# BenLangmead/bowtie2

Measured on NVIDIA H100. Metric: Mreads/s, higher is better.
Workload: dtype u64 popcount (FM rank) + s16x2 DPX (DP)

## Files before the change

### bowtie2_b200/csrc/xengine.cu

```cuda
#include <new>
#include <mutex>
#include <map>
#include <cstdio>
#include <cstddef>
#include <chrono>
#include <cstring>
#include <string>
#include <vector>
#include "dp_ungapped_device.cuh"
#include "dp_device.cuh"
#define XE_HD __device__
#include "xengine.cuh"
#include "xengine_shared.h"

template <typename OFF> int launch_dp_e2e(const DevIndex<OFF> &, const bt2g_scoring &, const DpLaunch &, int, cudaStream_t);
template <typename OFF> int launch_dp_local(const DevIndex<OFF> &, const bt2g_scoring &, const DpLaunch &, int, cudaStream_t);
template <typename OFF> void launch_exact_sweep2(const DevIndex<OFF> &, const uint64_t *, uint64_t, int, int, uint8_t *, uint64_t *, const uint64_t *, const uint32_t *, unsigned long long *, int, cudaStream_t, unsigned long long *, int);
void launch_pack_reads(const uint8_t *, const uint64_t *, uint64_t, int, uint64_t *, uint32_t *, cudaStream_t);
template <typename OFF> void launch_one_mm_sel(const DevIndex<OFF> &, const uint8_t *, const uint8_t *, const uint64_t *, uint64_t, const uint32_t *, const int32_t *, const uint8_t *, const bt2g_scoring &, int, bt2g_mm_hit *, int32_t *, cudaStream_t, bool);
template <typename OFF> void launch_seed_search_active(const DevIndex<OFF> &, const uint64_t *, uint64_t, int, int, const int32_t *, const int32_t *, const uint8_t *, uint64_t *, int32_t *, const uint64_t *, const uint32_t *, unsigned long long *, int, cudaStream_t);

extern "C" int bt2g_policy_align(const bt2g_policy_backend *, const bt2g_policy_params *, const bt2g_reads *, const char *const *,
                                 bt2g_read_result *, uint8_t *, uint32_t, bt2g_pair_result *, uint64_t *);

namespace {
using namespace xe;

#define XE_MM_MAXHITS 16
#define XE_TEV 96

struct XQueues {
	uint32_t nDpA, nDpM, nMm, nSeed, nDone, nFallback, nActive, pad1;
	unsigned long long cellsA, cellsM;
};

struct DpOut { bt2g_dp_problem *probs; bt2g_dp_summary *summ; bt2g_dp_cand *cands; bt2g_dp_aln *alns; uint8_t *ops; int maxCands, maxAlns, maxOps; };

struct XDev {
	const uint8_t *seq, *qual; const uint64_t *roff;
	const uint32_t *seeds;
	const uint64_t *packed; const uint32_t *nmask;
	const uint8_t *mine; const uint64_t *ee;
	const bt2g_mm_hit *mmHits; const int32_t *mmCounts;
	uint32_t *mmSel; int32_t *mmMinsc; uint8_t *mmMask;
	const uint64_t *ranges; const int32_t *nseeds; int maxSeeds;
	int32_t *seedInterval, *seedOffset; uint8_t *seedActive;
	DpOut A, M;
	XQueues *q;
	XUnit *units; uint8_t *status; uint64_t nUnits;
	bt2g_read_result *res; uint8_t *resOps; bt2g_pair_result *pairs; uint32_t resMaxOps;
};

template <typename OFF, bool K>
struct DevSvc {
	static constexpr bool kReport = K;
	const DevIndex<OFF> &ix; const bt2g_scoring &sc; const XDev &d;
	__device__ DevSvc(const DevIndex<OFF> &i, const bt2g_scoring &s, const XDev &dd) : ix(i), sc(s), d(dd) {}
	__device__ const uint8_t *codes(int read) const { return d.seq + d.roff[read]; }
	__device__ const uint8_t *quals(int read) const { return d.qual + d.roff[read]; }
	__device__ int rdlen(int read) const { return (int)(d.roff[read + 1] - d.roff[read]); }
	__device__ uint32_t randSeed(int read) const { return d.seeds[read]; }
	__device__ void sweep(int read, int mined[2], uint64_t tb[4]) const {
		mined[0] = d.mine[2 * (size_t)read]; mined[1] = d.mine[2 * (size_t)read + 1];
		for(int j = 0; j < 4; j++) tb[j] = d.ee[4 * (size_t)read + j];
	}
	__device__ int mmMax() const { return XE_MM_MAXHITS; }
// ... 44 lines not shown
	if(names) {
		const char *nm = names + i * (uint64_t)nameStride;
		for(uint32_t k = 0; k < nameStride && nm[k]; k++) { if(nm[k] == '/') break; rseed ^= (uint32_t)(unsigned char)nm[k] << ((k & 3) << 3); }
	} else {
		char buf[24]; int n = 0;
		uint64_t v = paired ? i >> 1 : i;
		char tmp[20]; int t = 0;
		do { tmp[t++] = (char)('0' + v % 10); v /= 10; } while(v);
		buf[n++] = 'r';
		while(t) buf[n++] = tmp[--t];
		for(int k = 0; k < n; k++) rseed ^= (uint32_t)(unsigned char)buf[k] << ((k & 3) << 3);
	}
	out[i] = rseed;
}

__global__ void k_xe_reset(XUnit *units, uint8_t *status, uint64_t nUnits, int paired) {
	const uint64_t i = blockIdx.x * (uint64_t)blockDim.x + threadIdx.x;
	if(i >= nUnits) return;
	x_unit_reset(units[i], (uint32_t)i, paired != 0);
	status[i] = 0;
}

__device__ __forceinline__ uint32_t agg_inc(uint32_t *ctr) {
	const unsigned act = __activemask();
	const unsigned peers = __match_any_sync(act, (unsigned long long)ctr);
	const int lane = threadIdx.x & 31, leader = __ffs(peers) - 1;
	uint32_t base = 0;
	if(lane == leader) base = atomicAdd(ctr, (uint32_t)__popc(peers));
	base = __shfl_sync(peers, base, leader);
	return base + (uint32_t)__popc(peers & ((1u << lane) - 1u));
}

template <typename OFF, int MINB, bool K>
__global__ void __launch_bounds__(128, MINB) k_xe_step(DevIndex<OFF> ix, bt2g_scoring sc, XParams P, XDev d, const uint32_t *activeIn, uint32_t *activeOut,
                                                       uint32_t nAct, int spread) {
	const uint64_t tt = blockIdx.x * (uint64_t)blockDim.x + threadIdx.x;
	const uint64_t t = tt >> spread;
	const bool valid = t < nAct && (tt & ((1u << spread) - 1u)) == 0;
	const uint64_t i = valid ? (activeIn ? activeIn[t] : t) : 0;
	int r = XR_DONE;
	if(valid) {
		XUnit &u = d.units[i];
		DevSvc<OFF, K> svc(ix, sc, d);
		r = x_step(P, u, svc);
		switch(r) {
		case XR_DP: case XR_DP_MATE: {
			const bool mate = r == XR_DP_MATE;
			const uint32_t slot = agg_inc(mate ? &d.q->nDpM : &d.q->nDpA);
			(mate ? d.M : d.A).probs[slot] = u.rqProb;
			u.dpSlot = (int32_t)slot;
			const unsigned long long cells = (unsigned long long)svc.rdlen((int)u.rqProb.read_idx) * (unsigned long long)(u.rqProb.refr - u.rqProb.refl + 1);
			atomicAdd(mate ? &d.q->cellsM : &d.q->cellsA, cells);
			break; }
		case XR_ONE_MM: {
			const uint32_t slot = agg_inc(&d.q->nMm);
			d.mmSel[slot] = (uint32_t)u.rqRead; d.mmMinsc[slot] = u.rqMinsc; d.mmMask[slot] = (uint8_t)((u.rqNofw ? 0 : 1) | (u.rqNorc ? 0 : 2));
			u.dpSlot = (int32_t)slot;
			break; }
		case XR_SEED:
			d.seedActive[u.rqRead] = 1; d.seedInterval[u.rqRead] = u.rqInterval; d.seedOffset[u.rqRead] = u.rqOffset;
			agg_inc(&d.q->nSeed);
			break;
		case XR_DONE: {
			d.status[i] = 1;
			agg_inc(&d.q->nDone);
			if(K) break;
			const uint64_t r0 = u.paired ? 2 * i : i; const int nr = u.paired ? 2 : 1;
			for(int k = 0; k < nr; k++) x_fill_result(u, k, svc.codes((int)(r0 + k)), d.res[r0 + k], d.resOps + (r0 + k) * (uint64_t)d.resMaxOps, d.resMaxOps);
			if(u.paired) { bt2g_pair_result pr; pr.pair_type = u.pairType; pr.kind = u.pairKind; pr.source = 0; pr.score_sum = (int32_t)u.scoreSum; pr.fraglen = u.fraglen; d.pairs[i] = pr; }
			break; }
		default:
			d.status[i] = 2;
			agg_inc(&d.q->nFallback);
			break;
		}
	}
	__syncwarp();
	const bool cont = valid && (r == XR_DP || r == XR_DP_MATE || r == XR_ONE_MM || r == XR_SEED);
	const unsigned m = __ballot_sync(0xffffffffu, cont);
	if(m) {
		const int lane = threadIdx.x & 31, leader = __ffs(m) - 1;
		uint32_t base = 0;
		if(lane == leader) base = atomicAdd(&d.q->nActive, (uint32_t)__popc(m));
		base = __shfl_sync(0xffffffffu, base, leader);
		if(cont) activeOut[base + (uint32_t)__popc(m & ((1u << lane) - 1u))] = (uint32_t)i;
	}
}

__global__ void __launch_bounds__(128) k_xe_report(XParams P, const XUnit *units, const uint8_t *status, uint64_t nUnits, const uint8_t *seq,
                                                   const uint64_t *roff, uint32_t maxPer, bt2g_read_result *res, uint8_t *ops, uint32_t maxOps,
                                                   bt2g_pair_result *pairs, uint32_t *nEntries, uint32_t *truncated) {
	const uint64_t w = (blockIdx.x * (uint64_t)blockDim.x + threadIdx.x) >> 5;
	const int lane = threadIdx.x & 31;
	if(w >= nUnits || status[w] != 1) return;
	const XUnit &u = units[w];
	const int n = x_report_count(u, P), nw = n < (int)maxPer ? n : (int)maxPer;
	if(lane == 0) {
		nEntries[w] = (uint32_t)nw;
		if(n > (int)maxPer && maxPer > 1) atomicOr(truncated, 1u);
	}
	const int per = u.paired ? 2 : 1;
	const uint64_t r0 = w * (uint64_t)per;
	const uint8_t *c0 = seq + roff[r0], *c1 = u.paired ? seq + roff[r0 + 1] : nullptr;
	for(int e = lane; e < (nw > 1 ? nw : 1); e += 32) {
		const uint64_t ent = w * (uint64_t)maxPer + (uint64_t)e;
		x_report_entry(u, P, e, c0, c1, res + ent * per, ops + ent * per * (uint64_t)maxOps, maxOps, u.paired ? pairs + ent : nullptr);
	}
}

struct DpWork {
	DpOut o{}; uint8_t *codes = nullptr; int32_t *lastH = nullptr; uint64_t *rawKeys = nullptr;
	int maxCol = 0, packed = 0, maxRaw = 0; uint64_t codeStride = 0, chunk = 0, numSlots = 0;
};

}

struct bt2g_xengine {
	bt2g_ctx *ctx = nullptr;
	bt2g_policy_params pp{};
	bt2g_scoring sc{};
	XParams P{}; XTables T;
	uint64_t maxUnits = 0, maxReads = 0, maxBases = 0; int maxLen = 0; uint32_t maxOps = 0;
	std::vector<void *> allocs;
	int32_t *dTabs = nullptr;
	XDev d{};
	DpWork A, M;
	uint64_t *packed = nullptr; uint32_t *nmask = nullptr; unsigned long long *nextTask = nullptr;
	uint32_t *active[2] = {nullptr, nullptr};
	uint8_t *dSeq = nullptr, *dQual = nullptr; uint64_t *dOff = nullptr; char *dNames = nullptr; uint32_t nameStrideCap = 0;
	XQueues *hq = nullptr;
	uint8_t *hStatus = nullptr;
	int sms = 148;
	cudaStream_t stream = nullptr;
	cudaStream_t streamHi = nullptr;
	bool ownStreams = false;
	int debug = 0;
	int bigSpread = 0;
	int stepOcc = 4;
	uint64_t stats[8] = {0, 0, 0, 0, 0, 0, 0, 0};
	float stageMs[12] = {0, 0, 0, 0, 0, 0, 0, 0, 0, 0, 0, 0};
	cudaEvent_t tev[2][XE_TEV]; int tevN[2] = {0, 0};
	cudaEvent_t evJoin = nullptr; int dpSideBySide = 1;
	uint64_t launches = 0;
	uint32_t maxPer = 0;
	bt2g_read_result *kRes = nullptr; uint8_t *kOps = nullptr; bt2g_pair_result *kPairs = nullptr; uint32_t *kN = nullptr, *kTrunc = nullptr;
	cudaEvent_t ev[8] = {nullptr, nullptr, nullptr, nullptr, nullptr, nullptr, nullptr, nullptr};
};

namespace {

template <typename T> int xalloc(bt2g_xengine *e, T *&ptr, uint64_t count) {
	void *v = nullptr;
	const cudaError_t err = cudaMalloc(&v, (count ? count : 1) * sizeof(T));
	if(err != cudaSuccess) { e->ctx->err = std::string("xengine cudaMalloc: ") + cudaGetErrorString(err); return -2; }
	e->allocs.push_back(v);
	ptr = (T *)v;
	return 0;
}

int setupDp(bt2g_xengine *e, DpWork &w, int maxCol, uint64_t cap, int maxCands, int maxAlns) {
	const bt2g_scoring &sc = e->sc;
// ... 28 lines not shown
	const DevIndex<OFF> ix = bt2g_dev_index<OFF>(e->ctx);
	e->launches += (!e->sc.local && w.packed == 3) ? 2 * ((n + w.chunk - 1) / w.chunk) : 1;
	return e->sc.local ? launch_dp_local<OFF>(ix, e->sc, L, e->maxLen, st) : launch_dp_e2e<OFF>(ix, e->sc, L, e->maxLen, st);
}

template <typename OFF>
int runBatch(bt2g_xengine *e, uint64_t nReads, const char *dNames, uint32_t nameStride, cudaStream_t st0) {
	cudaStream_t st = st0;
	bt2g_ctx *ctx = e->ctx;
	const bool paired = e->P.paired != 0;
	const uint64_t nUnits = paired ? nReads / 2 : nReads;
	const DevIndex<OFF> ix = bt2g_dev_index<OFF>(ctx);
	XDev &d = e->d;
	d.nUnits = nUnits;
	d.packed = e->packed; d.nmask = e->nmask;
	const unsigned T = 128;
	auto grid = [&](uint64_t m, unsigned t) { return (unsigned)((m + t - 1) / t); };
	for(int k = 0; k < 8; k++) e->stats[k] = 0;
	for(int k = 0; k < 12; k++) e->stageMs[k] = 0.f;
	e->tevN[0] = e->tevN[1] = 0;
	e->launches = 4;
	cudaEvent_t *ev = e->ev;
	auto lap = [&](int a, int b, int stage) { float ms = 0.f; if(cudaEventElapsedTime(&ms, ev[a], ev[b]) == cudaSuccess) e->stageMs[stage] += ms; };
	cudaEventRecord(ev[7], st);
	k_xe_seeds<<<grid(nReads, T), T, 0, st>>>(d.seq, d.qual, d.roff, nReads, dNames, nameStride, paired ? 1 : 0, e->P.seed, const_cast<uint32_t *>(d.seeds));
	k_xe_reset<<<grid(nUnits, T), T, 0, st>>>(d.units, d.status, nUnits, paired ? 1 : 0);
	launch_pack_reads(d.seq, d.roff, nReads, e->maxLen, e->packed, e->nmask, st);
	launch_exact_sweep2<OFF>(ix, d.roff, nReads, 0, 0, const_cast<uint8_t *>(d.mine), const_cast<uint64_t *>(d.ee), e->packed, e->nmask, e->nextTask, e->sms, st, nullptr,
	                         ix.extText ? 2 : 0 );
	BT2G_CUDA_TRY(ctx, cudaMemsetAsync(d.seedActive, 0, nReads, st));
	BT2G_CUDA_TRY(ctx, cudaGetLastError());
	uint64_t done = 0;
	uint32_t nActive = 0;
	cudaEventRecord(ev[0], st);
	for(uint64_t wave = 0;; wave++) {
		BT2G_CUDA_TRY(ctx, cudaMemsetAsync(d.q, 0, sizeof(XQueues), st));
		{
			const uint32_t nAct = wave == 0 ? (uint32_t)nUnits : nActive;
			const uint32_t *in = wave == 0 ? nullptr : e->active[wave & 1];
			uint32_t *out = e->active[(wave + 1) & 1];
			const int spread = (uint64_t)nAct * 32 <= (uint64_t)e->sms * 2048 * 4 ? 5 : e->bigSpread;
			const uint64_t nThr = (uint64_t)nAct << spread;
			if(e->maxPer) k_xe_step<OFF, 4, true><<<grid(nThr, 128), 128, 0, st>>>(ix, e->sc, e->P, d, in, out, nAct, spread);
			else if(e->stepOcc >= 8) k_xe_step<OFF, 8, false><<<grid(nThr, 128), 128, 0, st>>>(ix, e->sc, e->P, d, in, out, nAct, spread);
			else if(e->stepOcc >= 6) k_xe_step<OFF, 6, false><<<grid(nThr, 128), 128, 0, st>>>(ix, e->sc, e->P, d, in, out, nAct, spread);
			else k_xe_step<OFF, 4, false><<<grid(nThr, 128), 128, 0, st>>>(ix, e->sc, e->P, d, in, out, nAct, spread);
		}
		cudaEventRecord(ev[1], st);
		e->launches++;
		BT2G_CUDA_TRY(ctx, cudaMemcpyAsync(e->hq, d.q, sizeof(XQueues), cudaMemcpyDeviceToHost, st));
		BT2G_CUDA_TRY(ctx, cudaStreamSynchronize(st));
		if(wave == 0) lap(7, 0, 0); else { lap(2, 3, 2); lap(3, 4, 3); lap(4, 5, 4); lap(5, 0, 5); }
		for(int qi = 0; qi < 2; qi++) {
			for(int k = 0; k + 1 < e->tevN[qi]; k++) { float ms = 0.f; if(cudaEventElapsedTime(&ms, e->tev[qi][k], e->tev[qi][k + 1]) == cudaSuccess) e->stageMs[8 + (k & 1)] += ms; }
			e->tevN[qi] = 0;
		}
		lap(0, 1, 1);
		const XQueues q = *e->hq;
		if(e->debug) {
			float ms = 0.f; cudaEventElapsedTime(&ms, ev[0], ev[1]);
			fprintf(stderr, "[xengine] wave %llu: step %.3f ms; done %u fallback %u | dpA %u dpM %u mm %u seed %u\n", (unsigned long long)wave, ms, q.nDone, q.nFallback,
			        q.nDpA, q.nDpM, q.nMm, q.nSeed);
		}
		e->stats[0]++; e->stats[1] += q.nFallback; e->stats[2] += q.nDpA; e->stats[3] += q.nDpM; e->stats[4] += q.cellsA; e->stats[5] += q.cellsM;
		e->stats[6] += q.nMm; e->stats[7] += q.nSeed;
		e->launches += (q.nMm ? 1 : 0) + (q.nSeed ? 1 : 0);
		done += q.nDone + q.nFallback;
		nActive = q.nActive;
		if(done >= nUnits) break;
		if(e->ownStreams) st = (uint64_t)nActive * 32 <= (uint64_t)e->sms * 2048 * 4 ? e->streamHi : e->stream;
		if(q.nDpA + q.nDpM + q.nMm + q.nSeed == 0) { ctx->err = "xengine: units neither finished nor waiting"; return -5; }
		cudaEventRecord(ev[2], st);
		if(q.nMm) launch_one_mm_sel<OFF>(ix, d.seq, d.qual, d.roff, q.nMm, d.mmSel, d.mmMinsc, d.mmMask, e->sc, XE_MM_MAXHITS, const_cast<bt2g_mm_hit *>(d.mmHits), const_cast<int32_t *>(d.mmCounts), st,
		                                      ix.extText != 0);
		cudaEventRecord(ev[3], st);
		if(q.nSeed) {
			launch_seed_search_active<OFF>(ix, d.roff, nReads, e->P.seedLen, d.maxSeeds, d.seedInterval, d.seedOffset, d.seedActive, const_cast<uint64_t *>(d.ranges),
			                               const_cast<int32_t *>(d.nseeds), e->packed, e->nmask, e->nextTask, e->sms, st);
			BT2G_CUDA_TRY(ctx, cudaMemsetAsync(d.seedActive, 0, nReads, st));
		}
		cudaEventRecord(ev[4], st);
		const bool sideBySide = e->ownStreams && e->dpSideBySide && q.nDpA && q.nDpM && (uint64_t)(q.nDpA + q.nDpM) * 16 <= (uint64_t)e->sms * 2048;
		cudaStream_t stM = sideBySide ? (st == e->stream ? e->streamHi : e->stream) : st;
		if(launchDp<OFF>(e, e->A, q.nDpA, st)) { ctx->err = "xengine: DP launch rejected"; return -1; }
		cudaEventRecord(ev[5], st);
		if(launchDp<OFF>(e, e->M, q.nDpM, stM)) { ctx->err = "xengine: DP launch rejected"; return -1; }
		if(sideBySide) { cudaEventRecord(e->evJoin, stM); cudaStreamWaitEvent(st, e->evJoin, 0); }
		cudaEventRecord(ev[0], st);
		BT2G_CUDA_TRY(ctx, cudaGetLastError());
	}
	lap(7, 1, 7);
	return 0;
}

}

static int createEngine(bt2g_ctx *ctx, const bt2g_policy_params *pp, uint64_t maxUnits, uint32_t maxLen, uint32_t maxPer, bt2g_xengine **out) {
	BT2G_CUDA_TRY(ctx, cudaSetDevice(ctx->device));
	if(maxPer) {
		const uint64_t per = pp->paired ? 2 : 1, ents = maxUnits * (uint64_t)maxPer;
		const uint64_t need = ents * per * (sizeof(bt2g_read_result) + maxLen + 80) + (pp->paired ? ents * sizeof(bt2g_pair_result) : 0) + maxUnits * 4;
		size_t freeB = 0, totalB = 0;
		BT2G_CUDA_TRY(ctx, cudaMemGetInfo(&freeB, &totalB));
		if(need > freeB) {
			char msg[200];
			snprintf(msg, sizeof msg, "xengine: the -k / -a report arrays (%.2f GiB for %llu units x %u entries) do not fit the device's free memory (%.2f GiB)",
			         need / 1073741824.0, (unsigned long long)maxUnits, maxPer, freeB / 1073741824.0);
			ctx->err = msg;
			return -2;
		}
	}
	bt2g_xengine *e = new(std::nothrow) bt2g_xengine();
	if(!e) return -4;
	e->ctx = ctx; e->pp = *pp; e->maxLen = (int)maxLen; e->maxUnits = maxUnits;
	e->maxReads = pp->paired ? 2 * maxUnits : maxUnits; e->maxBases = e->maxReads * (uint64_t)maxLen;
	e->maxOps = maxLen + 80;
	cudaDeviceGetAttribute(&e->sms, cudaDevAttrMultiProcessorCount, ctx->device);
	if(const char *o = getenv("BT2G_XE_OCC")) e->stepOcc = atoi(o);
	if(getenv("BT2G_XE_DEBUG")) e->debug = 1;
	if(const char *o = getenv("BT2G_XE_DP_SERIAL")) e->dpSideBySide = atoi(o) ? 0 : 1;
	if(const char *o = getenv("BT2G_XE_SPREAD")) { e->bigSpread = atoi(o); if(e->bigSpread < 0 || e->bigSpread > 5) e->bigSpread = 0; }
	scoringFromParams(pp, &e->sc);
	ctx->scoring = e->sc;
	buildParams(pp, ctx->info.off_size, (int)maxLen, e->P, e->T);
	int rc = 0;
	const uint64_t nR = e->maxReads, nU = maxUnits;
	rc |= xalloc(e, e->dTabs, 4ull * (maxLen + 1));
	XDev &d = e->d;
	rc |= xalloc(e, e->dSeq, e->maxBases); rc |= xalloc(e, e->dQual, e->maxBases); rc |= xalloc(e, e->dOff, nR + 1);
	uint32_t *seeds; uint8_t *mine; uint64_t *ee;
	rc |= xalloc(e, seeds, nR); rc |= xalloc(e, mine, nR * 2); rc |= xalloc(e, ee, nR * 4);
	d.seeds = seeds; d.mine = mine; d.ee = ee;
	bt2g_mm_hit *mmHits; int32_t *mmCounts;
	rc |= xalloc(e, mmHits, nU * 4 * XE_MM_MAXHITS); rc |= xalloc(e, mmCounts, nU * 4);
	d.mmHits = mmHits; d.mmCounts = mmCounts;
	rc |= xalloc(e, d.mmSel, nU); rc |= xalloc(e, d.mmMinsc, nU); rc |= xalloc(e, d.mmMask, nU);
	{
		int minIval = 1 << 30;
		for(int l = 1; l <= (int)maxLen; l++) { minIval = std::min(minIval, std::min(e->T.ivalOne[l], e->T.ivalBoth[l])); }
		int ms = 1 + ((int)maxLen - std::min<int>(pp->seed_len, (int)maxLen)) / std::max(1, minIval) + 1;
		if(ms > XE_MAX_SEEDS) ms = XE_MAX_SEEDS + 1;
		d.maxSeeds = ms;
	}
	uint64_t *ranges; int32_t *nseeds;
	rc |= xalloc(e, ranges, nR * 2ull * d.maxSeeds * 4); rc |= xalloc(e, nseeds, nR);
	d.ranges = ranges; d.nseeds = nseeds;
	rc |= xalloc(e, d.seedInterval, nR); rc |= xalloc(e, d.seedOffset, nR); rc |= xalloc(e, d.seedActive, nR);
	rc |= xalloc(e, e->packed, (e->maxBases >> 5) + nR + 2); rc |= xalloc(e, e->nmask, (e->maxBases >> 5) + nR + 2); rc |= xalloc(e, e->nextTask, 1);
	rc |= xalloc(e, d.q, 1); rc |= xalloc(e, d.units, nU); rc |= xalloc(e, d.status, nU);
	rc |= xalloc(e, e->active[0], nU); rc |= xalloc(e, e->active[1], nU);
	if(maxPer) {
		const uint64_t ents = nU * (uint64_t)maxPer, rows = ents * (pp->paired ? 2 : 1);
		e->maxPer = maxPer;
		rc |= xalloc(e, e->kRes, rows); rc |= xalloc(e, e->kOps, rows * (uint64_t)e->maxOps); rc |= xalloc(e, e->kN, nU); rc |= xalloc(e, e->kTrunc, 1);
		if(pp->paired) rc |= xalloc(e, e->kPairs, ents);
		d.res = nullptr; d.resOps = nullptr; d.pairs = nullptr;
	} else {
		rc |= xalloc(e, d.res, nR); rc |= xalloc(e, d.resOps, nR * (uint64_t)e->maxOps); rc |= xalloc(e, d.pairs, nU);
	}
	d.resMaxOps = e->maxOps;
	if(!rc) {
		const int maxColA = (int)maxLen + 4 * 15 + 4;
		int gapMax = 15;
		for(int l = 1; l <= (int)maxLen; l++) { gapMax = std::max(gapMax, std::max(e->P.maxReadGaps(e->T.minsc[l], l), e->P.maxRefGaps(e->T.minsc[l], l))); }
		if(gapMax > 512) gapMax = 512;
		const uint64_t maxfrag = std::max<uint64_t>(pp->pe.maxfrag, maxLen);
		int maxColM = (int)std::min<uint64_t>(maxfrag + 2ull * maxLen + 2ull * gapMax + 16, 8000);
		const int maxCands = e->sc.local ? 16384 : 256, maxAlns = e->sc.local ? 32 : 8;
		rc |= setupDp(e, e->A, maxColA, nU, maxCands, maxAlns);
		if(pp->paired) rc |= setupDp(e, e->M, maxColM, nU, maxCands, maxAlns);
		else e->M = e->A;
		d.A = e->A.o; d.M = e->M.o;
	}
	cudaError_t err = cudaSuccess;
	if(!rc) {
		std::vector<int32_t> tabs(4ull * (maxLen + 1));
		for(uint32_t l = 0; l <= maxLen; l++) { tabs[l] = e->T.minsc[l]; tabs[(maxLen + 1) + l] = e->T.nceilRaw[l]; tabs[2 * (maxLen + 1) + l] = e->T.ivalOne[l]; tabs[3 * (maxLen + 1) + l] = e->T.ivalBoth[l]; }
		err = cudaMemcpy(e->dTabs, tabs.data(), tabs.size() * 4, cudaMemcpyHostToDevice);
		e->P.minscTab = e->dTabs; e->P.nceilRawTab = e->dTabs + (maxLen + 1); e->P.ivalOneTab = e->dTabs + 2 * (maxLen + 1); e->P.ivalBothTab = e->dTabs + 3 * (maxLen + 1);
		if(err == cudaSuccess) err = cudaHostAlloc((void **)&e->hq, sizeof(XQueues), cudaHostAllocDefault);
		if(err == cudaSuccess) err = cudaHostAlloc((void **)&e->hStatus, nU, cudaHostAllocDefault);
		for(int k = 0; k < 8 && err == cudaSuccess; k++) err = cudaEventCreate(&e->ev[k]);
		for(int k = 0; k < 2 * XE_TEV && err == cudaSuccess; k++) err = cudaEventCreate(&e->tev[k / XE_TEV][k % XE_TEV]);
// ... 263 lines not shown
```

### bowtie2_b200/csrc/xengine.cuh

```cuda
#pragma once
#include <stdint.h>
#include "../../include/bt2g.h"
#include "mapq_device.cuh"
#include "pe_device.cuh"

#ifndef XE_HD
#define XE_HD __host__ __device__
#endif
#define XE_HH __host__ __device__

namespace xe {

#define XE_MIN_I64 (-9223372036854775807LL - 1)
#define XE_BIG ((int64_t)1 << 62)
enum { EXHAUSTED = 1, FULFILLED, PERFECT, SOFT_LIMIT, HARD_LIMIT };
enum { XR_DONE = 0, XR_ONE_MM = 1, XR_SEED = 2, XR_DP = 3, XR_DP_MATE = 4, XR_FALLBACK = 5 };

#define XE_MAX_LEN    512
#define XE_ARENA      12288
#define XE_SEEN_IV    224
#define XE_EXR        8
#define XE_MM1        24
#define XE_MAX_SEEDS  64
#define XE_SATS       (2 * XE_MAX_SEEDS)
// ... 1337 lines not shown
			XE_CALL_EXT(5, stepExtUnpaired);
			if(u.xRet == FULFILLED) { if(u.usDone) u.rdone = 1; }
			else if(u.xRet == PERFECT || u.xRet == HARD_LIMIT) u.rdone = 1;
			if(!u.rdone && c.shNelt / c.shNonz < 300) u.rdone = 1;
		}
		finishRead();
		u.doneFlag = 1;
		return XR_DONE;
	}
	}
	XE_FB(u);
	return XR_FALLBACK;
}

template <typename Svc>
XE_HD void XEngine<Svc>::finishRead() {
	if(u.nus == 0) return;
	XSel buf[XE_LIST];
	for(int i = 0; i < u.nus; i++) { buf[i].score = x_aln(u, u.usAlns[i])->score; buf[i].idx = i; }
	x_select(buf, u.nus, u.rnd);
	u.resAligned[0] = 1; u.resAln[0] = u.usAlns[buf[0].idx];
	u.resHasXs[0] = u.nus > 1; u.resXs[0] = u.nus > 1 ? buf[1].score : 0;
	u.resMapq[0] = (int)mapq(x_aln(u, u.resAln[0])->score, u.resHasXs[0] != 0, u.resXs[0], P.minScore(u.m[0].rdlen), u.m[0].perfect);
	if(Svc::kReport && !P.mmode) x_permute_selected(buf, u.nus, u.usAlns, nullptr);
}

template <typename Svc>
XE_HD inline int x_step(const XParams &P, XUnit &u, Svc &svc) {
	XEngine<Svc> e(P, u, svc);
	const int r = u.paired ? e.stepPair() : e.stepRead();
	if(u.fallback) return XR_FALLBACK;
	return r;
}
XE_HD inline void x_unit_reset(XUnit &u, uint32_t id, bool paired) {
	u.pc = 0; u.pcExt = 0; u.fallback = 0; u.paired = paired; u.doneFlag = 0; u.id = id; u.arenaTop = 0; u.cur = 0;
	u.nents = 0; u.nsats = 0; u.nrands = 0; u.nseenPool = 0; u.nhitl = 0; u.natt = 0; u.attCursor = 0; u.dpSlot = -1;
	u.pairType = 0; u.pairKind = 5; u.scoreSum = 0; u.fraglen = 0;
	for(int k = 0; k < 2; k++) { u.resAligned[k] = 0; u.resHasXs[k] = 0; u.resMapq[k] = 0; u.resXs[k] = 0; u.resAln[k] = 0xffff; }
}

XE_HD inline void x_fill_row(const XAln *a, bool hasXs, int64_t xs, int mapq, const uint8_t *codes, bt2g_read_result &out, uint8_t *ops, uint32_t maxOps) {
	out.found = 0; out.score = 0; out.score2 = INT32_MIN; out.fw = 0; out.tidx = 0; out.refoff = 0; out.nops = 0; out.ndp = 0;
	out.trim_left = out.trim_right = 0; out.mapq = 0; out.pad = 0;
	if(!a) return;
	const int nops = x_aln_to_ops(a, codes, ops, maxOps);
	out.found = (a->nedits == 0 && a->ext() == a->rdlen) ? 2 : 1;
	out.score = a->score; if(hasXs) out.score2 = (int32_t)xs;
	out.fw = a->fw; out.tidx = (uint64_t)a->tidx; out.refoff = a->refoff; out.nops = nops;
	out.trim_left = a->trimLeft(); out.trim_right = a->rdlen - a->ext() - a->trimLeft();
	out.mapq = mapq; out.pad = a->refns;
}
XE_HD inline void x_fill_result(const XUnit &u, int k, const uint8_t *codes, bt2g_read_result &out, uint8_t *ops, uint32_t maxOps) {
	x_fill_row(u.resAligned[k] ? x_aln(u, u.resAln[k]) : nullptr, u.resHasXs[k] != 0, u.resXs[k], u.resMapq[k], codes, out, ops, maxOps);
}

XE_HD inline int x_report_secondaries(const XUnit &u, const XParams &P, int n) {
	if(P.mmode || n < 1) return 0;
	return (int)((int64_t)n < P.khits ? (int64_t)n : P.khits) - 1;
}
XE_HD inline int x_report_count(const XUnit &u, const XParams &P) {
	if(!u.paired) return u.resAligned[0] ? 1 + x_report_secondaries(u, P, u.nus) : 0;
	if(u.pairType == 1) return 1 + x_report_secondaries(u, P, u.nrs12);
	const int s0 = u.resAligned[0] ? x_report_secondaries(u, P, u.nrs1u) : 0, s1 = u.resAligned[1] ? x_report_secondaries(u, P, u.nrs2u) : 0;
	if(s0 + s1 == 0) return 1;
	return (u.resAligned[0] ? 1 + s0 : 1) + (u.resAligned[1] ? 1 + s1 : 1);
}
// ... 33 lines not shown
```

### bowtie2_b200/csrc/xengine_host.cpp

```cpp
#include <cmath>
#include <cstring>
#include <string>
#include <vector>
#include "../../include/bt2g.h"
#define __host__
#define __device__
#define __forceinline__ inline
#include "xengine.cuh"
#include "xengine_shared.h"

namespace xe {

static double funcF(int type, double C, double L, double x) {
	const double g = type == 1 ? 0.0 : type == 2 ? x : type == 3 ? std::sqrt(x) : std::log(x);
	return C + L * g;
}

void buildParams(const bt2g_policy_params *pp, int offSize, int maxLen, XParams &P, XTables &T) {
	memset(&P, 0, sizeof(P));
	P.local = pp->local; P.paired = pp->paired; P.all = pp->all_hits; P.mmode = pp->mmode; P.nofw = pp->nofw; P.norc = pp->norc;
	P.discord = pp->discord; P.mixed = pp->mixed;
	P.seedLen = pp->seed_len; P.seedRounds = pp->seed_rounds; P.streak = pp->dp_fail_streak;
	P.maxIters = 400; P.maxUg = 300; P.maxDp = 300; P.maxMateStreak = 10;
	P.khits = P.all ? XE_BIG : (pp->khits > 0 ? pp->khits : 1);
// ... 122 lines not shown
		const int32_t iv = rdlen(read) > 1 ? rdlen(read) : 1, of = rdoff;
		bt2g_seed_plan plan{seedlen, 1, 0, 0, &iv, &of};
		uint64_t ranges[8] = {0, 0, 0, 0, 0, 0, 0, 0};
		for(int j = 0; j < 4; j++) ranges[(fw ? 0 : 1) * 4 + j] = rng[j];
		uint8_t out[4] = {0, 0, 0, 0};
		rc |= be.extend_exact(be.ctx, &b, &plan, ranges, out); nCalls++;
		nlex = out[(fw ? 0 : 1) * 2]; nrex = out[(fw ? 0 : 1) * 2 + 1];
	}
	int ungapped(int read, bool fw, int64_t tidx, int64_t refoff, int64_t tlen, int64_t minsc, bt2g_ungapped_result &r) {
		uint64_t o2[2]; bt2g_reads b = one(read, o2);
		bt2g_ungapped_problem p{}; p.read_idx = 0; p.fw = fw; p.tidx = (uint64_t)tidx; p.refoff = refoff; p.reflen = (uint64_t)tlen; p.minsc = (int32_t)minsc; p.ohang = 0;
		rc |= be.ungapped(be.ctx, &b, &p, 1, &r, nullptr, 0); nCalls++;
		if(r.status == 1) {
			const int32_t cnt = rdlen(read);
			stretch.assign((size_t)cnt, 4);
			const uint64_t ti = (uint64_t)tidx;
			rc |= be.get_stretch(be.ctx, &ti, &refoff, &cnt, 1, cnt, stretch.data()); nCalls++;
			stTidx = tidx; stOff = refoff;
		}
		return r.status;
	}
	int refChar(int64_t tidx, int64_t off) const {
		const int64_t k = off - stOff;
		if(tidx != stTidx || k < 0 || k >= (int64_t)stretch.size()) return 4;
		return stretch[(size_t)k];
	}
};

}

extern "C" int bt2g_policy_align(const bt2g_policy_backend *, const bt2g_policy_params *, const bt2g_reads *, const char *const *,
                                 bt2g_read_result *, uint8_t *, uint32_t, bt2g_pair_result *, uint64_t *);

static int alignHost(const bt2g_policy_backend *be, const bt2g_policy_params *pp, const bt2g_reads *reads, const char *const *names, uint32_t maxPer,
                     bt2g_read_result *res, uint8_t *ops, uint32_t maxOps, bt2g_pair_result *pairs, uint32_t *nEntries, uint64_t *stats) {
	using namespace xe;
	if(!be || !pp || !reads || !res || !ops || (pp->paired && (!pairs || (reads->n_reads & 1))) || (maxPer && !nEntries)) return -1;
	bool truncated = false;
	int maxLen = 1;
	for(uint64_t i = 0; i < reads->n_reads; i++) { const int l = (int)(reads->off[i + 1] - reads->off[i]); if(l > maxLen) maxLen = l; }
	XParams P; XTables T;
	buildParams(pp, be->off_size, maxLen, P, T);
	HostSvc svc(*be, P, reads, names);
	const size_t units = P.paired ? reads->n_reads / 2 : reads->n_reads;
	std::vector<XUnit> ubuf(1);
	XUnit &u = ubuf[0];
	uint64_t nReq = 0, nFallback = 0;
	for(size_t id = 0; id < units; id++) {
		x_unit_reset(u, (uint32_t)id, P.paired != 0);
		int r;
		for(;;) {
			r = x_step(P, u, svc);
			if(r == XR_DONE || r == XR_FALLBACK) break;
			nReq++;
			if(r == XR_ONE_MM) svc.answerOneMm(u);
			else if(r == XR_SEED) svc.answerSeed(u);
			else if(r == XR_DP) svc.answerDp(u, false);
			else if(r == XR_DP_MATE) svc.answerDp(u, true);
			u.dpSlot = 0;
			if(svc.rc) return -2;
		}
		if(svc.rc) return -2;
		const size_t r0 = P.paired ? 2 * id : id, nr = P.paired ? 2 : 1;
		if(r == XR_FALLBACK) {
			nFallback++;
			bt2g_reads sub; sub.n_reads = nr; sub.seq = reads->seq + reads->off[r0]; sub.qual = reads->qual + reads->off[r0];
			uint64_t off3[3] = {0, reads->off[r0 + 1] - reads->off[r0], nr == 2 ? reads->off[r0 + 2] - reads->off[r0] : 0};
			sub.off = off3;
			const char *nm[2] = {names ? names[r0] : nullptr, (names && nr == 2) ? names[r0 + 1] : nullptr};
			if(maxPer) {
				const size_t e0 = id * (size_t)maxPer;
				const int rc2 = P.paired ? bt2g_policy_align_pairs_k(be, pp, &sub, names ? nm : nullptr, maxPer, res + 2 * e0, ops + 2 * e0 * (size_t)maxOps, maxOps, pairs + e0, nEntries + id, nullptr)
				                         : bt2g_policy_align_k(be, pp, &sub, names ? nm : nullptr, maxPer, res + e0, ops + e0 * (size_t)maxOps, maxOps, nEntries + id, nullptr);
				if(rc2 < 0) return rc2;
				truncated = truncated || rc2 == 1;
				continue;
			}
			bt2g_pair_result pr{};
			const int rc2 = bt2g_policy_align(be, pp, &sub, names ? nm : nullptr, res + r0, ops + r0 * (size_t)maxOps, maxOps, P.paired ? &pr : nullptr, nullptr);
			if(rc2 < 0) return rc2;
			if(P.paired) pairs[id] = pr;
			continue;
		}
		if(maxPer) {
// ... 31 lines not shown
```

### bowtie2_b200/lib.py

```python
from __future__ import annotations

import ctypes as C
import os
from typing import Optional

import numpy as np

_HERE = os.path.dirname(os.path.abspath(__file__))
_LIB = None

OFFMASK = np.uint64(0xFFFFFFFFFFFFFFFF)


class Bt2GpuError(RuntimeError):
    pass


def library_path() -> str:
    return os.path.join(_HERE, "libbt2g.so")


class _IndexHost(C.Structure):
    _fields_ = [
        ("off_size", C.c_int32), ("line_rate", C.c_int32), ("off_rate", C.c_int32), ("ftab_chars", C.c_int32),
# ... 895 lines not shown
                  "rec_off": int(d.n_recs), "rec_len": int(d.n_recs)}
        p = getattr(d, name)
        p = p if isinstance(p, int) else C.cast(p, C.c_void_p).value
        if not p:
            return None
        if name in counts:
            dt = np.uint32 if osz == 4 else np.uint64
            nbytes = counts[name] * osz
        else:
            dt = np.uint8
            if name in ("ebwt_fw", "ebwt_bw"):
                nbytes = nsides * side
            elif name == "rec_first":
                nbytes = int(d.n_recs)
            else:
                rl = self.array("rec_len")
                nbytes = (int(rl.sum()) + 3) >> 2
        buf = (C.c_uint8 * nbytes).from_address(p)
        return np.frombuffer(buf, dtype=dt).copy()

    def close(self):
        if getattr(self, "_h", None):
            self._lib.bt2g_index_file_close(self._h)
            self._h = None

    def __del__(self):
        try:
            self.close()
        except Exception:
            pass


EXPORTS += ["bt2g_policy_align", "bt2g_policy_align_k", "bt2g_policy_align_pairs_k", "bt2g_policy_backend_gpu", "bt2g_xengine_align_host",
            "bt2g_xengine_align_host_k"]
_CB = C.CFUNCTYPE
_vp = C.c_void_p


class _PolicyBackend(C.Structure):
    _fields_ = [("ctx", _vp),
                ("exact_sweep", _CB(C.c_int, _vp, _vp, C.c_int, C.c_int, _vp, _vp)),
                ("seed_search", _CB(C.c_int, _vp, _vp, _vp, _vp, _vp)),
                ("one_mm", _CB(C.c_int, _vp, _vp, _vp, _vp, C.c_int32, _vp, _vp)),
                ("extend_exact", _CB(C.c_int, _vp, _vp, _vp, _vp, _vp)),
                ("resolve", _CB(C.c_int, _vp, _vp, _vp, C.c_uint64, C.c_int, _vp, _vp, _vp, _vp, _vp)),
                ("get_stretch", _CB(C.c_int, _vp, _vp, _vp, _vp, C.c_uint64, C.c_int32, _vp)),
                ("ungapped", _CB(C.c_int, _vp, _vp, _vp, C.c_uint64, _vp, _vp, C.c_uint32)),
                ("dp_extend", _CB(C.c_int, _vp, _vp, _vp, C.c_uint64, C.c_int32, C.c_int32, C.c_int32, _vp, _vp, _vp, _vp)),
                ("off_size", C.c_int32), ("reserved", C.c_int32)]


class _PePolicyS(C.Structure):
    _fields_ = [("pol", C.c_int32), ("flags", C.c_int32), ("maxfrag", C.c_uint64), ("minfrag", C.c_uint64)]


class _PolicyParams(C.Structure):
    _fields_ = [("local", C.c_int32), ("paired", C.c_int32), ("seed_len", C.c_int32), ("seed_rounds", C.c_int32), ("dp_fail_streak", C.c_int32),
                ("ival_type", C.c_int32), ("ival_const", C.c_double), ("ival_coeff", C.c_double),
                ("smin_type", C.c_int32), ("smin_const", C.c_double), ("smin_coeff", C.c_double),
                ("nceil_const", C.c_double), ("nceil_coeff", C.c_double), ("khits", C.c_int64), ("mhits", C.c_int64),
                ("mmode", C.c_int32), ("all_hits", C.c_int32), ("nofw", C.c_int32), ("norc", C.c_int32), ("discord", C.c_int32),
                ("mixed", C.c_int32), ("seed", C.c_uint32), ("max_inflight", C.c_int32),
                ("match_bonus", C.c_int32), ("mmp_max", C.c_int32), ("mmp_min", C.c_int32), ("n_pen", C.c_int32),
                ("rdgap_const", C.c_int32), ("rdgap_linear", C.c_int32), ("rfgap_const", C.c_int32), ("rfgap_linear", C.c_int32),
                ("pe", _PePolicyS), ("host_threads", C.c_int32), ("reserved", C.c_int32)]


# ... 356 lines not shown
```

### include/bt2g.h

```cpp
#ifndef BT2G_H_
#define BT2G_H_
#include <stdint.h>
#include <stddef.h>

#ifdef __cplusplus
extern "C" {
#endif

typedef struct bt2g_ctx bt2g_ctx;

int         bt2g_create(int device, bt2g_ctx **out);
void        bt2g_destroy(bt2g_ctx *ctx);
const char *bt2g_last_error(const bt2g_ctx *ctx);
int         bt2g_abi_version(void);

typedef struct {
	int32_t  off_size;
	int32_t  line_rate, off_rate, ftab_chars;
	uint64_t len;
	uint64_t n_pat, n_frag;
	uint64_t z_off_fw, z_off_bw;
	uint64_t fchr[5];
	const void    *plen;
	const void    *rstarts;
// ... 320 lines not shown
	int64_t mhits;
	int32_t mmode, all_hits;
	int32_t nofw, norc, discord, mixed;
	uint32_t seed; int32_t max_inflight;
	int32_t match_bonus, mmp_max, mmp_min, n_pen, rdgap_const, rdgap_linear, rfgap_const, rfgap_linear;
	bt2g_pe_policy pe;
	int32_t host_threads;
	int32_t reserved;
} bt2g_policy_params;

int bt2g_policy_align(const bt2g_policy_backend *be, const bt2g_policy_params *prm, const bt2g_reads *reads, const char *const *names,
                      bt2g_read_result *res, uint8_t *ops, uint32_t max_ops, bt2g_pair_result *pairs, uint64_t *stats);

int bt2g_policy_align_k(const bt2g_policy_backend *be, const bt2g_policy_params *prm, const bt2g_reads *reads, const char *const *names,
                        uint32_t max_per_read, bt2g_read_result *res, uint8_t *ops, uint32_t max_ops, uint32_t *n_reported,
                        uint64_t *stats);
int bt2g_policy_align_pairs_k(const bt2g_policy_backend *be, const bt2g_policy_params *prm, const bt2g_reads *reads, const char *const *names,
                              uint32_t max_per_pair, bt2g_read_result *res, uint8_t *ops, uint32_t max_ops, bt2g_pair_result *pairs,
                              uint32_t *n_entries, uint64_t *stats);

typedef struct bt2g_xengine bt2g_xengine;
int  bt2g_xengine_create(bt2g_ctx *ctx, const bt2g_policy_params *prm, uint64_t max_units , uint32_t max_len,
                         bt2g_xengine **out);
void bt2g_xengine_destroy(bt2g_xengine *e);
int  bt2g_xengine_align(bt2g_xengine *e, const bt2g_reads *reads, const char *names, uint32_t name_stride, bt2g_read_result *res,
                        uint8_t *ops, uint32_t max_ops, bt2g_pair_result *pairs, uint64_t *stats);
int  bt2g_xengine_run_dev(bt2g_xengine *e, const uint8_t *d_seq, const uint8_t *d_qual, const uint64_t *d_off, uint64_t n_reads,
                          const char *d_names, uint32_t name_stride, void *stream, uint64_t *stats);
int  bt2g_xengine_results_dev(bt2g_xengine *e, bt2g_read_result **res, uint8_t **ops, uint32_t *max_ops, bt2g_pair_result **pairs);
int  bt2g_xengine_streams(bt2g_xengine *e, void **stream, void **stream_hi);
int  bt2g_xengine_stage_ms(bt2g_xengine *e, float *ms, uint64_t *launches);
int  bt2g_xengine_align_host(const bt2g_policy_backend *be, const bt2g_policy_params *prm, const bt2g_reads *reads, const char *const *names,
                             bt2g_read_result *res, uint8_t *ops, uint32_t max_ops, bt2g_pair_result *pairs, uint64_t *stats);

int  bt2g_xengine_create_k(bt2g_ctx *ctx, const bt2g_policy_params *prm, uint64_t max_units, uint32_t max_len, uint32_t max_per_unit,
                           bt2g_xengine **out);
int  bt2g_xengine_align_k(bt2g_xengine *e, const bt2g_reads *reads, const char *names, uint32_t name_stride, bt2g_read_result *res,
                          uint8_t *ops, uint32_t max_ops, bt2g_pair_result *pairs, uint32_t *n_entries, uint64_t *stats);
int  bt2g_xengine_results_k_dev(bt2g_xengine *e, bt2g_read_result **res, uint8_t **ops, uint32_t *max_ops, bt2g_pair_result **pairs,
                                uint32_t **n_entries, uint32_t *max_per_unit);
int  bt2g_xengine_align_host_k(const bt2g_policy_backend *be, const bt2g_policy_params *prm, const bt2g_reads *reads, const char *const *names,
                               uint32_t max_per_unit, bt2g_read_result *res, uint8_t *ops, uint32_t max_ops, bt2g_pair_result *pairs,
                               uint32_t *n_entries, uint64_t *stats);

int bt2g_fastq_parse_mt(const char *text, uint64_t len, uint64_t max_reads, uint64_t max_bases, uint8_t *seq, uint8_t *qual,
                        uint64_t *off, char *names, uint32_t name_stride, uint64_t *n_reads, uint64_t *consumed, int threads);

int bt2g_fastq_parse_pairs_mt(const char *text1, uint64_t len1, const char *text2, uint64_t len2, uint64_t max_pairs, uint64_t max_bases,
                              uint8_t *seq, uint8_t *qual, uint64_t *off, char *names, uint32_t name_stride, uint64_t *n_pairs,
                              uint64_t *consumed1, uint64_t *consumed2, int threads);

typedef int (*bt2g_stream_align_fn)(void *engine, const bt2g_reads *reads, const char *names, uint32_t name_stride, bt2g_read_result *res,
                                    uint8_t *ops, uint32_t max_ops, bt2g_pair_result *pairs, uint64_t *stats);
typedef struct {
	void *user;
	int (*next_block)(void *user, const char **text1, uint64_t *len1, const char **text2, uint64_t *len2);
	int (*write)(void *user, const char *sam, uint64_t len);
	int64_t (*read)(void *user, int mate, char *dst, uint64_t cap);
} bt2g_stream_io;
typedef struct {
	int32_t  paired, parse_threads, format_threads, depth ;
	uint64_t max_units;
	uint32_t max_len, max_ops, name_stride, count_flags;
	uint64_t chunk_bytes;
	void    *solo_engine;
	uint64_t solo_max_units;
// ... 10 lines not shown
```

Measured before the change: 2.695.

## Bucket active units by resume key to reduce warp divergence in step kernel

Instead of compacting continuing units into one active list, each unit is appended to a per-resume-key bucket (pc/pcExt), and the next wave reads buckets in a fixed cost order so that warps hold units resuming at the same program point. This targets divergence in the state-machine step kernel. It adds a per-thread bucket lookup loop, 24 separate atomic counters, and active buffers that are 24 times larger. Debug counters and a host trace hook are added for measuring keys per warp.

Result: faster. 2.754 (median of 6 runs) (+2.2%).

```diff
diff --git a/bowtie2_b200/csrc/xengine.cu b/bowtie2_b200/csrc/xengine.cu
--- a/bowtie2_b200/csrc/xengine.cu
+++ b/bowtie2_b200/csrc/xengine.cu
@@ -30,8 +30,16 @@
 #define XE_TEV 96
 
 struct XQueues {
-	uint32_t nDpA, nDpM, nMm, nSeed, nDone, nFallback, nActive, pad1;
+	uint32_t nDpA, nDpM, nMm, nSeed, nDone, nFallback, warps, keysInWarps;
 	unsigned long long cellsA, cellsM;
+	uint32_t nKey[XE_KEYS];
+};
+
+struct XActive {
+	const uint32_t *in; uint32_t *out;
+	uint64_t stride;
+	uint32_t n; int nReg, group, debug;
+	uint32_t start[XE_KEYS + 1]; uint8_t reg[XE_KEYS];
 };
 
 struct DpOut { bt2g_dp_problem *probs; bt2g_dp_summary *summ; bt2g_dp_cand *cands; bt2g_dp_aln *alns; uint8_t *ops; int maxCands, maxAlns, maxOps; };
@@ -142,17 +150,30 @@
 }
 
 template <typename OFF, int MINB, bool K>
-__global__ void __launch_bounds__(128, MINB) k_xe_step(DevIndex<OFF> ix, bt2g_scoring sc, XParams P, XDev d, const uint32_t *activeIn, uint32_t *activeOut,
-                                                       uint32_t nAct, int spread) {
+__global__ void __launch_bounds__(128, MINB) k_xe_step(DevIndex<OFF> ix, bt2g_scoring sc, XParams P, XDev d, XActive A, int spread) {
 	const uint64_t tt = blockIdx.x * (uint64_t)blockDim.x + threadIdx.x;
 	const uint64_t t = tt >> spread;
-	const bool valid = t < nAct && (tt & ((1u << spread) - 1u)) == 0;
-	const uint64_t i = valid ? (activeIn ? activeIn[t] : t) : 0;
-	int r = XR_DONE;
+	const bool valid = t < A.n && (tt & ((1u << spread) - 1u)) == 0;
+	uint64_t i = valid ? t : 0;
+	if(valid && A.in) {
+		int g = 0;
+		while(g + 1 < A.nReg && t >= A.start[g + 1]) g++;
+		i = A.in[A.reg[g] * A.stride + (t - A.start[g])];
+	}
+	if(A.debug) {
+		const unsigned vm = __ballot_sync(0xffffffffu, valid);
+		const int key = valid ? x_resume_key(d.units[i]) : -1;
+		const unsigned peers = __match_any_sync(0xffffffffu, key);
+		const bool lead = valid && (threadIdx.x & 31) == __ffs(peers) - 1;
+		const unsigned lm = __ballot_sync(0xffffffffu, lead);
+		if((threadIdx.x & 31) == 0 && vm) { atomicAdd(&d.q->warps, 1u); atomicAdd(&d.q->keysInWarps, (uint32_t)__popc(lm)); }
+	}
+	int key = -1;
 	if(valid) {
 		XUnit &u = d.units[i];
 		DevSvc<OFF, K> svc(ix, sc, d);
-		r = x_step(P, u, svc);
+		const int r = x_step(P, u, svc);
+		if(r == XR_DP || r == XR_DP_MATE || r == XR_ONE_MM || r == XR_SEED) key = A.group ? x_resume_key(u) : 0;
 		switch(r) {
 		case XR_DP: case XR_DP_MATE: {
 			const bool mate = r == XR_DP_MATE;
@@ -186,15 +207,7 @@
 		}
 	}
 	__syncwarp();
-	const bool cont = valid && (r == XR_DP || r == XR_DP_MATE || r == XR_ONE_MM || r == XR_SEED);
-	const unsigned m = __ballot_sync(0xffffffffu, cont);
-	if(m) {
-		const int lane = threadIdx.x & 31, leader = __ffs(m) - 1;
-		uint32_t base = 0;
-		if(lane == leader) base = atomicAdd(&d.q->nActive, (uint32_t)__popc(m));
-		base = __shfl_sync(0xffffffffu, base, leader);
-		if(cont) activeOut[base + (uint32_t)__popc(m & ((1u << lane) - 1u))] = (uint32_t)i;
-	}
+	if(key >= 0) A.out[key * A.stride + agg_inc(&d.q->nKey[key])] = (uint32_t)i;
 }
 
 __global__ void __launch_bounds__(128) k_xe_report(XParams P, const XUnit *units, const uint8_t *status, uint64_t nUnits, const uint8_t *seq,
@@ -237,6 +250,7 @@
 	DpWork A, M;
 	uint64_t *packed = nullptr; uint32_t *nmask = nullptr; unsigned long long *nextTask = nullptr;
 	uint32_t *active[2] = {nullptr, nullptr};
+	int group = 1;
 	uint8_t *dSeq = nullptr, *dQual = nullptr; uint64_t *dOff = nullptr; char *dNames = nullptr; uint32_t nameStrideCap = 0;
 	XQueues *hq = nullptr;
 	uint8_t *hStatus = nullptr;
@@ -331,19 +345,21 @@
 	BT2G_CUDA_TRY(ctx, cudaGetLastError());
 	uint64_t done = 0;
 	uint32_t nActive = 0;
+	XActive A{};
+	A.stride = e->maxUnits; A.group = e->group; A.debug = e->debug;
 	cudaEventRecord(ev[0], st);
 	for(uint64_t wave = 0;; wave++) {
 		BT2G_CUDA_TRY(ctx, cudaMemsetAsync(d.q, 0, sizeof(XQueues), st));
 		{
-			const uint32_t nAct = wave == 0 ? (uint32_t)nUnits : nActive;
-			const uint32_t *in = wave == 0 ? nullptr : e->active[wave & 1];
-			uint32_t *out = e->active[(wave + 1) & 1];
-			const int spread = (uint64_t)nAct * 32 <= (uint64_t)e->sms * 2048 * 4 ? 5 : e->bigSpread;
-			const uint64_t nThr = (uint64_t)nAct << spread;
-			if(e->maxPer) k_xe_step<OFF, 4, true><<<grid(nThr, 128), 128, 0, st>>>(ix, e->sc, e->P, d, in, out, nAct, spread);
-			else if(e->stepOcc >= 8) k_xe_step<OFF, 8, false><<<grid(nThr, 128), 128, 0, st>>>(ix, e->sc, e->P, d, in, out, nAct, spread);
-			else if(e->stepOcc >= 6) k_xe_step<OFF, 6, false><<<grid(nThr, 128), 128, 0, st>>>(ix, e->sc, e->P, d, in, out, nAct, spread);
-			else k_xe_step<OFF, 4, false><<<grid(nThr, 128), 128, 0, st>>>(ix, e->sc, e->P, d, in, out, nAct, spread);
+			A.n = wave == 0 ? (uint32_t)nUnits : nActive;
+			A.in = wave == 0 ? nullptr : e->active[wave & 1];
+			A.out = e->active[(wave + 1) & 1];
+			const int spread = (uint64_t)A.n * 32 <= (uint64_t)e->sms * 2048 * 4 ? 5 : e->bigSpread;
+			const uint64_t nThr = (uint64_t)A.n << spread;
+			if(e->maxPer) k_xe_step<OFF, 4, true><<<grid(nThr, 128), 128, 0, st>>>(ix, e->sc, e->P, d, A, spread);
+			else if(e->stepOcc >= 8) k_xe_step<OFF, 8, false><<<grid(nThr, 128), 128, 0, st>>>(ix, e->sc, e->P, d, A, spread);
+			else if(e->stepOcc >= 6) k_xe_step<OFF, 6, false><<<grid(nThr, 128), 128, 0, st>>>(ix, e->sc, e->P, d, A, spread);
+			else k_xe_step<OFF, 4, false><<<grid(nThr, 128), 128, 0, st>>>(ix, e->sc, e->P, d, A, spread);
 		}
 		cudaEventRecord(ev[1], st);
 		e->launches++;
@@ -358,14 +374,17 @@
 		const XQueues q = *e->hq;
 		if(e->debug) {
 			float ms = 0.f; cudaEventElapsedTime(&ms, ev[0], ev[1]);
-			fprintf(stderr, "[xengine] wave %llu: step %.3f ms; done %u fallback %u | dpA %u dpM %u mm %u seed %u\n", (unsigned long long)wave, ms, q.nDone, q.nFallback,
-			        q.nDpA, q.nDpM, q.nMm, q.nSeed);
+			fprintf(stderr, "[xengine] wave %llu: step %.3f ms; %u units, %.2f resume keys per warp; done %u fallback %u | dpA %u dpM %u mm %u seed %u\n",
+			        (unsigned long long)wave, ms, A.n, q.warps ? (double)q.keysInWarps / q.warps : 0.0, q.nDone, q.nFallback, q.nDpA, q.nDpM, q.nMm, q.nSeed);
 		}
 		e->stats[0]++; e->stats[1] += q.nFallback; e->stats[2] += q.nDpA; e->stats[3] += q.nDpM; e->stats[4] += q.cellsA; e->stats[5] += q.cellsM;
 		e->stats[6] += q.nMm; e->stats[7] += q.nSeed;
 		e->launches += (q.nMm ? 1 : 0) + (q.nSeed ? 1 : 0);
 		done += q.nDone + q.nFallback;
-		nActive = q.nActive;
+		static const uint8_t byCost[XE_KEYS] = {16, 21, 22, 13, 14, 5, 6, 8, 0, 1, 2, 3, 4, 7, 9, 10, 11, 12, 15, 17, 18, 19, 20, 23};
+		nActive = 0; A.nReg = 0;
+		for(int j = 0; j < XE_KEYS; j++) { const int k = byCost[j]; if(q.nKey[k]) { A.reg[A.nReg] = (uint8_t)k; A.start[A.nReg++] = nActive; nActive += q.nKey[k]; } }
+		A.start[A.nReg] = nActive;
 		if(done >= nUnits) break;
 		if(e->ownStreams) st = (uint64_t)nActive * 32 <= (uint64_t)e->sms * 2048 * 4 ? e->streamHi : e->stream;
 		if(q.nDpA + q.nDpM + q.nMm + q.nSeed == 0) { ctx->err = "xengine: units neither finished nor waiting"; return -5; }
@@ -417,6 +436,7 @@
 	cudaDeviceGetAttribute(&e->sms, cudaDevAttrMultiProcessorCount, ctx->device);
 	if(const char *o = getenv("BT2G_XE_OCC")) e->stepOcc = atoi(o);
 	if(getenv("BT2G_XE_DEBUG")) e->debug = 1;
+	if(const char *o = getenv("BT2G_XE_GROUP")) e->group = atoi(o) ? 1 : 0;
 	if(const char *o = getenv("BT2G_XE_DP_SERIAL")) e->dpSideBySide = atoi(o) ? 0 : 1;
 	if(const char *o = getenv("BT2G_XE_SPREAD")) { e->bigSpread = atoi(o); if(e->bigSpread < 0 || e->bigSpread > 5) e->bigSpread = 0; }
 	scoringFromParams(pp, &e->sc);
@@ -447,7 +467,7 @@
 	rc |= xalloc(e, d.seedInterval, nR); rc |= xalloc(e, d.seedOffset, nR); rc |= xalloc(e, d.seedActive, nR);
 	rc |= xalloc(e, e->packed, (e->maxBases >> 5) + nR + 2); rc |= xalloc(e, e->nmask, (e->maxBases >> 5) + nR + 2); rc |= xalloc(e, e->nextTask, 1);
 	rc |= xalloc(e, d.q, 1); rc |= xalloc(e, d.units, nU); rc |= xalloc(e, d.status, nU);
-	rc |= xalloc(e, e->active[0], nU); rc |= xalloc(e, e->active[1], nU);
+	rc |= xalloc(e, e->active[0], nU * XE_KEYS); rc |= xalloc(e, e->active[1], nU * XE_KEYS);
 	if(maxPer) {
 		const uint64_t ents = nU * (uint64_t)maxPer, rows = ents * (pp->paired ? 2 : 1);
 		e->maxPer = maxPer;
diff --git a/bowtie2_b200/csrc/xengine.cuh b/bowtie2_b200/csrc/xengine.cuh
--- a/bowtie2_b200/csrc/xengine.cuh
+++ b/bowtie2_b200/csrc/xengine.cuh
@@ -1393,6 +1393,13 @@
 	if(u.fallback) return XR_FALLBACK;
 	return r;
 }
+
+#define XE_KEYS 24
+XE_HD inline int x_resume_key(const XUnit &u) {
+	const int pc = u.pc, k = pc * 4 + ((pc & 1) ? u.pcExt : 0);
+	return k < XE_KEYS ? k : 0;
+}
+
 XE_HD inline void x_unit_reset(XUnit &u, uint32_t id, bool paired) {
 	u.pc = 0; u.pcExt = 0; u.fallback = 0; u.paired = paired; u.doneFlag = 0; u.id = id; u.arenaTop = 0; u.cur = 0;
 	u.nents = 0; u.nsats = 0; u.nrands = 0; u.nseenPool = 0; u.nhitl = 0; u.natt = 0; u.attCursor = 0; u.dpSlot = -1;
diff --git a/bowtie2_b200/csrc/xengine_host.cpp b/bowtie2_b200/csrc/xengine_host.cpp
--- a/bowtie2_b200/csrc/xengine_host.cpp
+++ b/bowtie2_b200/csrc/xengine_host.cpp
@@ -178,6 +178,13 @@
 extern "C" int bt2g_policy_align(const bt2g_policy_backend *, const bt2g_policy_params *, const bt2g_reads *, const char *const *,
                                  bt2g_read_result *, uint8_t *, uint32_t, bt2g_pair_result *, uint64_t *);
 
+static void (*gTrace)(void *, uint64_t, int32_t) = nullptr;
+static void *gTraceUser = nullptr;
+
+extern "C" void bt2g_xengine_host_trace(void (*fn)(void *user, uint64_t unit, int32_t key), void *user) {
+	gTrace = fn; gTraceUser = user;
+}
+
 static int alignHost(const bt2g_policy_backend *be, const bt2g_policy_params *pp, const bt2g_reads *reads, const char *const *names, uint32_t maxPer,
                      bt2g_read_result *res, uint8_t *ops, uint32_t maxOps, bt2g_pair_result *pairs, uint32_t *nEntries, uint64_t *stats) {
 	using namespace xe;
@@ -196,6 +203,7 @@
 		x_unit_reset(u, (uint32_t)id, P.paired != 0);
 		int r;
 		for(;;) {
+			if(gTrace) gTrace(gTraceUser, id, x_resume_key(u));
 			r = x_step(P, u, svc);
 			if(r == XR_DONE || r == XR_FALLBACK) break;
 			nReq++;
diff --git a/bowtie2_b200/lib.py b/bowtie2_b200/lib.py
--- a/bowtie2_b200/lib.py
+++ b/bowtie2_b200/lib.py
@@ -951,7 +951,7 @@
 
 
 EXPORTS += ["bt2g_policy_align", "bt2g_policy_align_k", "bt2g_policy_align_pairs_k", "bt2g_policy_backend_gpu", "bt2g_xengine_align_host",
-            "bt2g_xengine_align_host_k"]
+            "bt2g_xengine_align_host_k", "bt2g_xengine_host_trace"]
 _CB = C.CFUNCTYPE
 _vp = C.c_void_p
 
diff --git a/include/bt2g.h b/include/bt2g.h
--- a/include/bt2g.h
+++ b/include/bt2g.h
@@ -376,6 +376,7 @@
 int  bt2g_xengine_stage_ms(bt2g_xengine *e, float *ms, uint64_t *launches);
 int  bt2g_xengine_align_host(const bt2g_policy_backend *be, const bt2g_policy_params *prm, const bt2g_reads *reads, const char *const *names,
                              bt2g_read_result *res, uint8_t *ops, uint32_t max_ops, bt2g_pair_result *pairs, uint64_t *stats);
+void bt2g_xengine_host_trace(void (*fn)(void *user, uint64_t unit, int32_t key), void *user);
 
 int  bt2g_xengine_create_k(bt2g_ctx *ctx, const bt2g_policy_params *prm, uint64_t max_units, uint32_t max_len, uint32_t max_per_unit,
                            bt2g_xengine **out);
```
